# rgcgithub/regenie

Measured on NVIDIA H100. Metric: step1_level0_snps_per_sec, higher is better.
Workload: dtype int8 Gram + int8 prediction (both exact integer sums) + tf32x3 factorisation + f64 refinement / statistics

## Files before the change

### regenie_b200/csrc/chol_mixed.cu

```cuda
#include <algorithm>

#include "gemm_dmma.cuh"
#include "kernels.cuh"

namespace rg {

namespace {

constexpr int PT = 128;
constexpr int PLD = 132;
constexpr int PB = 32;
constexpr int kMxRowsPerCta = 64;

__device__ __forceinline__ void blk_nt(float (&acc)[PB], const float* __restrict__ Arow, const float* __restrict__ Bt, int plen) {
  for (int p0 = 0; p0 < plen; p0 += 4) {
    const float4 a = *reinterpret_cast<const float4*>(Arow + p0);
#pragma unroll
    for (int n = 0; n < PB; ++n) {
      const float4 b = *reinterpret_cast<const float4*>(Bt + n * PLD + p0);
      acc[n] = fmaf(a.x, b.x, acc[n]);
      acc[n] = fmaf(a.y, b.y, acc[n]);
      acc[n] = fmaf(a.z, b.z, acc[n]);
      acc[n] = fmaf(a.w, b.w, acc[n]);
    }
// ... 200 lines not shown
#pragma unroll
    for (int p = 0; p < PMAX; ++p) acc[a][p] = 0.0;
  double2 an2[4];
#pragma unroll
  for (int a = 0; a < 4; ++a) an2[a] = *reinterpret_cast<const double2*>(a0 + (int64_t)a * n + lane * 2);
  for (int j = lane * 2; j < n; j += 64) {
    double2 av[4];
#pragma unroll
    for (int a = 0; a < 4; ++a) av[a] = an2[a];
    if (j + 64 < n) {
#pragma unroll
      for (int a = 0; a < 4; ++a) an2[a] = *reinterpret_cast<const double2*>(a0 + (int64_t)a * n + j + 64);
    }
#pragma unroll
    for (int p = 0; p < PMAX; ++p) {
      if (p < P) {
        const double2 b = *reinterpret_cast<const double2*>(rs_sm + p * n + j);
#pragma unroll
        for (int a = 0; a < 4; ++a) acc[a][p] = fma(av[a].x, b.x, fma(av[a].y, b.y, acc[a][p]));
      }
    }
  }
#pragma unroll
  for (int a = 0; a < 4; ++a)
#pragma unroll
    for (int p = 0; p < PMAX; ++p) {
#pragma unroll
      for (int o = 16; o > 0; o >>= 1) acc[a][p] += __shfl_xor_sync(0xffffffffu, acc[a][p], o);
    }
  if (lane == 0) {
#pragma unroll
    for (int a = 0; a < 4; ++a)
#pragma unroll
      for (int p = 0; p < PMAX; ++p)
        if (p < P)
          rvec[((int64_t)m * Pp + p) * n + i0 + a] = bvec[((int64_t)f * Pp + p) * n + i0 + a] - lam * rs_sm[p * n + i0 + a] - acc[a][p];
  }
  }
}


constexpr int RF_ROWS = 64;
constexpr int RF_NV = 64;

__global__ void __launch_bounds__(256)
mx_residual_fused_kernel(const double* __restrict__ Af, const double* __restrict__ lambda, int R, const double* __restrict__ bvec,
                         const double* __restrict__ xvec, double* __restrict__ rvec, int n, int P, int Pp, int nmat, int step,
                         const unsigned int* __restrict__ conv, float tol) {
  __shared__ double As[64 * DM_LD], Bs[64 * DM_LD];
  const int f = blockIdx.y;
  if (step > 1) {
    bool all_done = true;
    for (int r = 0; r < R; ++r) all_done = all_done && mx_finished(conv, nmat, f * R + r, step - 1, tol);
    if (all_done) return;
  }
  const int NV = R * P;
  const int row0 = blockIdx.x * RF_ROWS;
  const int lrow = threadIdx.x >> 2, lp = (threadIdx.x & 3) * 4;
  const bool vb = lrow < NV;
  const double* ap = Af + ((int64_t)f * n + row0 + lrow) * n + lp;
  const double* bp = xvec + ((int64_t)(f * R + (vb ? lrow / P : 0)) * Pp + (vb ? lrow % P : 0)) * n + lp;
  DmmaAcc acc;
  gemm_tile_nt_dmma_ptr(ap, true, bp, vb, n, acc, As, Bs);
#pragma unroll
  for (int j = 0; j < 4; ++j)
#pragma unroll
    for (int e = 0; e < 2; ++e) {
      const int vec = dm_col(j) + e;
      if (vec < NV) {
        const int r = vec / P, p = vec % P, m = f * R + r;
        const double lam = lambda[r];
#pragma unroll
        for (int i = 0; i < 2; ++i) {
          const int row = row0 + dm_row(i);
          const int64_t o = ((int64_t)m * Pp + p) * n + row;
          rvec[o] = bvec[((int64_t)f * Pp + p) * n + row] - lam * xvec[o] - acc.c[i][j][e];
        }
      }
    }
}

constexpr int TS_STAGES = 6;
constexpr int TS_SUB = 32;
constexpr int TS_STAGE_BYTES = TS_SUB * PT * 4;
constexpr int TS_VP = 12;
constexpr int TS_CW = 16;

__device__ __forceinline__ uint32_t ts_smem_u32(const void* p) { return (uint32_t)__cvta_generic_to_shared(p); }
__device__ __forceinline__ void ts_mbar_wait(uint32_t bar, uint32_t parity) {
  uint32_t done = 0, spins = 0;
  while (true) {
    asm volatile(
        "{\n\t.reg .pred p;\n\t"
        "mbarrier.try_wait.parity.shared::cta.b64 p, [%1], %2;\n\t"
        "selp.u32 %0, 1, 0, p;\n\t}"
        : "=r"(done) : "r"(bar), "r"(parity) : "memory");
    if (done) break;
    if (++spins > (1u << 28)) __trap();
  }
}

template <int PMAX>
__global__ void __launch_bounds__(32 * (TS_CW + 1))
mx_trisolve_kernel(const __grid_constant__ CUtensorMap tmL, const __grid_constant__ CUtensorMap tmM,
                   const __grid_constant__ CUtensorMap tmMT, const double* __restrict__ rvec, int64_t r_mat_stride,
                   int r_mat_div, double* __restrict__ xvec, int n, int P, int Pp, int nmat, int step,
                   unsigned int* __restrict__ conv, float tol) {
  constexpr int TS_PARTS = TS_CW / 4;
  constexpr int TS_CPP = TS_SUB / TS_PARTS;
  constexpr int TS_THREADS = 32 * (TS_CW + 1);
  extern __shared__ uint8_t ts_raw[];
  const int m = blockIdx.x;
  if (step > 1 && mx_finished(conv, nmat, m, step - 1, tol)) return;
  const uint32_t raw = ts_smem_u32(ts_raw);
  const uint32_t base = (raw + 127u) & ~127u;
  uint8_t* gen = ts_raw + (base - raw);
  float* tiles = reinterpret_cast<float*>(gen);
  float* v = reinterpret_cast<float*>(gen + TS_STAGES * TS_STAGE_BYTES);
  float* sbuf = v + (size_t)n * TS_VP;
  float* comb = sbuf + PT * TS_VP;
  uint64_t* bars = reinterpret_cast<uint64_t*>(comb + (TS_PARTS - 1) * PT * TS_VP);
  const uint32_t full_bar = ts_smem_u32(bars), empty_bar = ts_smem_u32(bars + TS_STAGES);
  const int warp = threadIdx.x >> 5, lane = threadIdx.x & 31;
  const int nt = n / PT;
  if (threadIdx.x == 0) {
    for (int s = 0; s < TS_STAGES; ++s) {
      asm volatile("mbarrier.init.shared::cta.b64 [%0], %1;" ::"r"(full_bar + 8 * s), "r"(1) : "memory");
      asm volatile("mbarrier.init.shared::cta.b64 [%0], %1;" ::"r"(empty_bar + 8 * s), "r"(TS_CW) : "memory");
    }
    asm volatile("fence.mbarrier_init.release.cluster;" ::: "memory");
    asm volatile("fence.proxy.async.shared::cta;" ::: "memory");
  }
  const double* r = rvec + (int64_t)(r_mat_div > 0 ? m / r_mat_div : m) * r_mat_stride;
  for (int e = threadIdx.x; e < n * TS_VP; e += TS_THREADS) {
    const int i = e / TS_VP, p = e % TS_VP;
    v[e] = p < P ? (float)r[(int64_t)p * n + i] : 0.f;
  }
  __syncthreads();

  if (warp == TS_CW) {
    if (lane == 0) {
      asm volatile("prefetch.tensormap [%0];" ::"l"(&tmL) : "memory");
      asm volatile("prefetch.tensormap [%0];" ::"l"(&tmM) : "memory");
      asm volatile("prefetch.tensormap [%0];" ::"l"(&tmMT) : "memory");
      int it = 0;
      auto push = [&](const CUtensorMap* tm, int c0, int c1) {
        const int s = it % TS_STAGES;
        const uint32_t ph = (it / TS_STAGES) & 1;
        ts_mbar_wait(empty_bar + 8 * s, ph ^ 1);
        asm volatile("mbarrier.arrive.expect_tx.shared::cta.b64 _, [%0], %1;" ::"r"(full_bar + 8 * s), "r"(TS_STAGE_BYTES) : "memory");
        asm volatile(
            "cp.async.bulk.tensor.2d.shared::cluster.global.mbarrier::complete_tx::bytes [%0], [%1, {%3, %4}], [%2];"
            ::"r"(base + s * TS_STAGE_BYTES), "l"(tm), "r"(full_bar + 8 * s), "r"(c0), "r"(c1) : "memory");
        ++it;
      };
      for (int sweep = 0; sweep < 2; ++sweep)
        for (int kk = 0; kk < nt; ++kk) {
          const int k = sweep == 0 ? kk : nt - 1 - kk;
          const int j0 = sweep == 0 ? 0 : k + 1, j1 = sweep == 0 ? k : nt;
          for (int j = j0; j < j1; ++j)
            for (int sub = 0; sub < PT / TS_SUB; ++sub) push(&tmL, k * PT, m * n + j * PT + sub * TS_SUB);
          for (int sub = 0; sub < PT / TS_SUB; ++sub)
            push(sweep == 0 ? &tmMT : &tmM, 0, (m * nt + k) * PT + sub * TS_SUB);
        }
    }
    return;
  }

  const int half = warp >> 2;
  const int row = (warp & 3) * 32 + lane;
  int it = 0;
  float acc[PMAX];
  auto consume = [&](const float* vec ) {
    const int s = it % TS_STAGES;
    const uint32_t ph = (it / TS_STAGES) & 1;
    ts_mbar_wait(full_bar + 8 * s, ph);
    const float* t = tiles + (size_t)s * (TS_STAGE_BYTES / 4) + (size_t)(half * TS_CPP) * PT + row;
    const float* y = vec + (size_t)(half * TS_CPP) * TS_VP;
#pragma unroll
    for (int c = 0; c < TS_CPP; ++c) {
      const float tv = t[(size_t)c * PT];
      const float4 y0 = *reinterpret_cast<const float4*>(y + c * TS_VP);
      const float4 y1 = *reinterpret_cast<const float4*>(y + c * TS_VP + 4);
      const float4 y2 = *reinterpret_cast<const float4*>(y + c * TS_VP + 8);
      const float yy[12] = {y0.x, y0.y, y0.z, y0.w, y1.x, y1.y, y1.z, y1.w, y2.x, y2.y, y2.z, y2.w};
#pragma unroll
      for (int p = 0; p < PMAX; ++p) acc[p] = fmaf(tv, yy[p], acc[p]);
    }
    __syncwarp();
    if (lane == 0) asm volatile("mbarrier.arrive.shared::cta.b64 _, [%0];" ::"r"(empty_bar + 8 * s) : "memory");
    ++it;
  };
  auto consumer_sync = [&]() { asm volatile("bar.sync 1, %0;" ::"n"(32 * TS_CW) : "memory"); };

  for (int sweep = 0; sweep < 2; ++sweep)
    for (int kk = 0; kk < nt; ++kk) {
      const int k = sweep == 0 ? kk : nt - 1 - kk;
      const int j0 = sweep == 0 ? 0 : k + 1, j1 = sweep == 0 ? k : nt;
#pragma unroll
      for (int p = 0; p < PMAX; ++p) acc[p] = 0.f;
      for (int j = j0; j < j1; ++j)
        for (int sub = 0; sub < PT / TS_SUB; ++sub) consume(v + (size_t)(j * PT + sub * TS_SUB) * TS_VP);
      if (half > 0) {
#pragma unroll
        for (int p = 0; p < PMAX; ++p) comb[((half - 1) * PT + row) * TS_VP + p] = acc[p];
      }
      consumer_sync();
      if (half == 0) {
#pragma unroll
        for (int p = 0; p < PMAX; ++p) {
          float sum = acc[p];
#pragma unroll
          for (int h = 0; h < TS_PARTS - 1; ++h) sum += comb[(h * PT + row) * TS_VP + p];
          sbuf[row * TS_VP + p] = v[(size_t)(k * PT + row) * TS_VP + p] - sum;
        }
      }
      consumer_sync();
#pragma unroll
      for (int p = 0; p < PMAX; ++p) acc[p] = 0.f;
      for (int sub = 0; sub < PT / TS_SUB; ++sub) consume(sbuf + (size_t)(sub * TS_SUB) * TS_VP);
      if (half > 0) {
#pragma unroll
        for (int p = 0; p < PMAX; ++p) comb[((half - 1) * PT + row) * TS_VP + p] = acc[p];
      }
      consumer_sync();
      if (half == 0) {
#pragma unroll
        for (int p = 0; p < PMAX; ++p) {
          float sum = acc[p];
#pragma unroll
          for (int h = 0; h < TS_PARTS - 1; ++h) sum += comb[(h * PT + row) * TS_VP + p];
          v[(size_t)(k * PT + row) * TS_VP + p] = sum;
        }
      }
      consumer_sync();
    }

  float dmax = 0.f, xmax = 0.f;
  for (int e = threadIdx.x; e < P * n; e += 32 * TS_CW) {
    const int p = e / n, i = e % n;
    double* xp = xvec + ((int64_t)m * Pp + p) * n + i;
    const float dx = v[(size_t)i * TS_VP + p];
    const double xn = (step == 0 ? 0.0 : *xp) + (double)dx;
    *xp = xn;
    dmax = (fabsf(dx) <= 3.0e38f) ? fmaxf(dmax, fabsf(dx)) : __int_as_float(0x7f800000);
    xmax = fmaxf(xmax, fabsf((float)xn));
  }
  if (step > 0) {
#pragma unroll
    for (int o = 16; o > 0; o >>= 1) {
      dmax = fmaxf(dmax, __shfl_xor_sync(0xffffffffu, dmax, o));
      xmax = fmaxf(xmax, __shfl_xor_sync(0xffffffffu, xmax, o));
    }
    if (lane == 0) {
      atomicMax(conv + ((int64_t)step * nmat + m) * 2, __float_as_uint(dmax));
      atomicMax(conv + ((int64_t)step * nmat + m) * 2 + 1, __float_as_uint(xmax));
    }
  }
}

__global__ void mx_final_check_kernel(const unsigned int* __restrict__ conv, int nmat, int steps, float tol,
                                      unsigned int* __restrict__ fail_flag) {
  const int m = blockIdx.x * blockDim.x + threadIdx.x;
  if (m >= nmat) return;
  bool ok = mx_finished(conv, nmat, m, steps, tol);
  for (int s = 1; s <= steps; ++s) {
    const float dx = __uint_as_float(conv[((int64_t)s * nmat + m) * 2]);
    if (!(dx == dx) || !(fabsf(dx) <= 3.0e38f)) ok = false;
  }
  if (!ok) atomicOr(fail_flag, 1u);
}

struct MxPlan {
  int n = 0, nt = 0;
  DevBuf<int4> tiles;
  std::vector<int2> upd, trsm;
};

static void build_plan(MxPlan& pl, int n) {
  pl.n = n;
  const int nt = n / PT;
  pl.nt = nt;
  std::vector<int4> all;
  pl.upd.clear(); pl.trsm.clear();
  for (int k = 0; k < nt; ++k) {
    int2 u{(int)all.size(), 0};
    for (int i = k; i < nt; ++i) all.push_back(make_int4(i, k, 0, 4 * k));
    u.y = (int)all.size() - u.x;
    pl.upd.push_back(u);
    int2 t{(int)all.size(), 0};
    for (int i = k + 1; i < nt; ++i) all.push_back(make_int4(i, k, 4 * k, 4));
    t.y = (int)all.size() - t.x;
    pl.trsm.push_back(t);
  }
  pl.tiles.alloc(all.size());
  RG_CUDA(cudaMemcpy(pl.tiles.p, all.data(), all.size() * sizeof(int4), cudaMemcpyHostToDevice));
}

struct MixedSolver::Impl {
  int n = 0, nmat = 0, K = 0, R = 0, Pp = 0;
  DevBuf<float> Lplain, Mplain, MTplain, Ap;
  DevBuf<unsigned int> conv;
  CUtensorMap tmL, tmM, tmAp;
  CUtensorMap tmLpl, tmMpl, tmMTpl;
  MxPlan plan;
};

MixedSolver::MixedSolver() : impl(new Impl()) {}
MixedSolver::~MixedSolver() { delete impl; }

int MixedSolver::dim_for(int bs) {
  int n = PT;
  while (n < bs) n *= 2;
  return n <= 2048 ? n : 0;
}

void MixedSolver::prepare(int n, int K, int R, int Pp) {
  Impl& d = *impl;
  const int nmat = K * R;
  if (d.n == n && d.nmat == nmat && d.Pp == Pp) return;
  RG_CHECK(n % PT == 0 && n >= PT && ((n / PT) & (n / PT - 1)) == 0 && n <= 2048,
           "mixed solver: dimension must be 128 * 2^k <= 2048");
  d.n = n; d.nmat = nmat; d.K = K; d.R = R; d.Pp = Pp;
  d.Lplain.alloc((size_t)nmat * n * n);
  d.Mplain.alloc((size_t)nmat * n * PT);
  d.MTplain.alloc((size_t)nmat * n * PT);
  make_f32_rows_tensor_map(&d.tmLpl, d.Lplain.p, n, (int64_t)nmat * n, PT, TS_SUB);
  make_f32_rows_tensor_map(&d.tmMpl, d.Mplain.p, PT, (int64_t)nmat * n, PT, TS_SUB);
  make_f32_rows_tensor_map(&d.tmMTpl, d.MTplain.p, PT, (int64_t)nmat * n, PT, TS_SUB);
  RG_CUDA(cudaMemset(d.Lplain.p, 0, (size_t)nmat * n * n * 4));
  d.conv.alloc((size_t)(kMxMaxSteps + 1) * nmat * 2);
  make_tf32_operand_tensor_map(&d.tmL, d.Lplain.p, n, n, nmat);
  make_tf32_operand_tensor_map(&d.tmM, d.Mplain.p, PT, n, nmat);
  d.Ap.alloc((size_t)K * n * n);
  RG_CUDA(cudaMemset(d.Ap.p, 0, (size_t)K * n * n * 4));
  make_tf32_operand_tensor_map(&d.tmAp, d.Ap.p, n, n, K);
  build_plan(d.plan, n);
}

static int rhs_chunk(int n) { return std::max(1, std::min(12, (int)(98304 / (8 * (size_t)n)))); }

int MixedSolver::launches_per_solve(int n, int steps, int P) {
  const int nt = n / PT;
  const int nch = (P + rhs_chunk(n) - 1) / rhs_chunk(n);
  return 3 * nt - 1 + nch * (1 + 2 * steps) + 1;
}

void MixedSolver::solve(const double* Af, const double* lambda, const double* bvec, double* xvec, double* rvec, int P,
                        int steps, float tol, unsigned int* fail_flag, cudaStream_t s, bool first_col_ready) {
  Impl& d = *impl;
  const int n = d.n, nmat = d.nmat, nt = d.plan.nt;
  RG_CHECK(n > 0, "mixed solver: prepare() first");
  RG_CHECK(P <= d.Pp, "mixed solver: more right-hand sides than the row pitch");
  RG_CHECK(steps >= 1 && steps <= kMxMaxSteps, "mixed solver: bad step count");
  const size_t potrf_smem = ((size_t)3 * PT * PLD + PT + 2 * PB) * sizeof(float);
  ensure_dyn_smem(reinterpret_cast<const void*>(potrf128_kernel), potrf_smem);
  ensure_dyn_smem(reinterpret_cast<const void*>(mx_residual_kernel<12>), 98304);
  ensure_dyn_smem(reinterpret_cast<const void*>(mx_residual_kernel<10>), 98304);
  RG_CHECK(n <= 2048, "mixed solver: n <= 2048");
  const size_t sm_t = (size_t)TS_STAGES * TS_STAGE_BYTES + ((size_t)n + (1 + TS_CW / 4) * PT) * TS_VP * sizeof(float) + 2 * TS_STAGES * 8 + 256;
  ensure_dyn_smem(reinterpret_cast<const void*>(mx_trisolve_kernel<12>), sm_t);
  ensure_dyn_smem(reinterpret_cast<const void*>(mx_trisolve_kernel<10>), sm_t);
  RG_CUDA(cudaMemsetAsync(d.conv.p, 0, d.conv.n * sizeof(unsigned int), s));
  const int4* tl = d.plan.tiles.p;
  Tf32GemmEpilogue e0{};
  e0.n = n; e0.out_mat_stride = (int64_t)n * n; e0.out = d.Lplain.p;
  for (int k = 0; k < nt; ++k) {
    Tf32GemmEpilogue e = e0;
    e.c_chunks = 4; e.c_mat_div = d.R;
    e.diag_add = lambda; e.diag_mod = d.R;
    if (!(k == 0 && first_col_ready)) launch_tf32x3_gemm(d.tmL, d.tmL, tl + d.plan.upd[k].x, d.plan.upd[k].y, nmat, e, s, &d.tmAp);
    potrf128_kernel<<<nmat, 256, potrf_smem, s>>>(d.Lplain.p, d.Mplain.p, d.MTplain.p, n, k, fail_flag);
    if (d.plan.trsm[k].y > 0) {
      Tf32GemmEpilogue t = e0;
      t.mirror = 1;
      t.b_cols_local = 1;
      launch_tf32x3_gemm(d.tmL, d.tmM, tl + d.plan.trsm[k].x, d.plan.trsm[k].y, nmat, t, s);
    }
  }
  dim3 grid(n / kMxRowsPerCta, nmat);
  const int pc = rhs_chunk(n);
  for (int st = 0; st <= steps; ++st)
    for (int p0 = 0; p0 < P; p0 += pc) {
      const int np = std::min(pc, P - p0);
      const size_t sm_r = (size_t)np * n * sizeof(double);
      const int64_t o = (int64_t)p0 * n;
      auto tri = [&](const double* rv, int64_t rs, int rdiv, int step) {
#define RG_TRI(PM) mx_trisolve_kernel<PM><<<nmat, 32 * (TS_CW + 1), sm_t, s>>>(d.tmLpl, d.tmMpl, d.tmMTpl, rv, rs, rdiv, xvec + o, n, np, d.Pp, nmat, step, d.conv.p, tol)
        if (np <= 10) RG_TRI(10);
        else RG_TRI(12);
#undef RG_TRI
      };
      if (st == 0) {
        tri(bvec + o, (int64_t)d.Pp * n, d.R, 0);
      } else {
        if (d.R * np <= RF_NV && n % RF_ROWS == 0)
          mx_residual_fused_kernel<<<dim3(n / RF_ROWS, d.K), 256, 0, s>>>(Af, lambda, d.R, bvec + o, xvec + o, rvec + o, n, np, d.Pp, nmat, st, d.conv.p, tol);
        else if (np <= 10) mx_residual_kernel<10><<<grid, 256, sm_r, s>>>(Af, lambda, d.R, bvec + o, xvec + o, rvec + o, n, np, d.Pp, nmat, st, d.conv.p, tol);
        else mx_residual_kernel<12><<<grid, 256, sm_r, s>>>(Af, lambda, d.R, bvec + o, xvec + o, rvec + o, n, np, d.Pp, nmat, st, d.conv.p, tol);
        tri(rvec + o, (int64_t)d.Pp * n, 0, st);
      }
    }
  mx_final_check_kernel<<<(nmat + 63) / 64, 64, 0, s>>>(d.conv.p, nmat, steps, tol, fail_flag);
}

float* MixedSolver::a_planes() { return impl->Ap.p; }
float* MixedSolver::l_planes() { return impl->Lplain.p; }

const float* MixedSolver::debug_planes(int which) const {
  switch (which) {
    case 2: return impl->Lplain.p;
    case 3: return impl->Mplain.p;
    default: return nullptr;
  }
}

}
```

### regenie_b200/csrc/kernels.cuh

```cuda
#pragma once
#include "common.cuh"

namespace rg {

constexpr int kMaxFolds = 16;
constexpr int kMaxCov = 64;
constexpr int kMaxRidge = 8;
constexpr int kMaxPhenoTile = 8;
constexpr int kLimbs = 9;
constexpr int kLimbsI8 = 5;
constexpr int kLimbQI8 = 50;

void launch_partial_sum(const double* part, int nchunks, int64_t per, double* out, cudaStream_t s);

__device__ __forceinline__ uint32_t miss_bits(uint32_t w) { return w & (w >> 1) & 0x55555555u; }
struct BedMissOut {
  const int4* ctile = nullptr;
  int nct = 0;
  int rows_p = 0;
  unsigned long long* total = nullptr;
  unsigned long long cap = 0;
  int2* seg = nullptr;
  int32_t* list = nullptr;
  uint32_t* gt = nullptr;
// ... 20 lines not shown
  double *gty_f, *rhs;
  unsigned long long* err_slot;
  long long err_base;
};

struct AssembleArgs {
  int bs, rows_p, nC, C, K, R, loocv;
  const float* zz;
  int64_t ldz, zz_fold_stride;
  const double *mu, *inv_sd, *Bv, *Af, *Qf;
  const double* lambda;
  double* cm;
  int64_t cm_stride;
  int ldc;
  float* planes = nullptr;
  float* lplanes = nullptr;
};

void launch_l0_stats(const uint32_t* gp, int64_t npad, const double* xy, int cpp, const int4* chunks,
                     int nchunks, int rows_p, int32_t* cnt_part, double* sum_part, cudaStream_t s);
void launch_l0_fold_reduce(const int32_t* cnt_part, const double* sum_part, int rows_p, int cpp,
                           const int2* fold_chunks, int K, int32_t* cnt_fold, double* sum_fold,
                           cudaStream_t s);
void launch_l0_snp_finalize(const SnpFinalizeArgs& a, cudaStream_t s);
void launch_l0_assemble(const AssembleArgs& a, const double* rhs, int P, int Ppad, int nmat, cudaStream_t s);

void make_gram_tensor_map(CUtensorMap* tm, const uint8_t* z, int64_t npad, int rows2);
constexpr int kStatQ = 14;
constexpr int kStatOnesRow = 126;
void launch_l0_xy_digits(const double* xy, int cpp, int ncol, int64_t npad, const uint8_t* is_real, double* scale,
                         uint8_t* D, cudaStream_t s);
void launch_l0_stats_finish(const float* T, int ldt, int64_t t_fold_stride, const float* zz, int ldz,
                            int64_t zz_fold_stride, int rows_p, int cpp, int ncol, int K, const double* scale,
                            int32_t* cnt_fold, double* sum_fold, cudaStream_t s);
void gram_tile_list(int rows2, std::vector<int2>& tiles);
void stat_tile_list(int zrows, int drows, int bn, std::vector<int2>& tiles);
struct ZPlanes {
  uint32_t lut[3];
};
constexpr uint32_t kPlaneG = 0x00100800u;
constexpr uint32_t kPlaneG2 = 0x00200800u;
constexpr uint32_t kPlaneMiss = 0x08000000u;
constexpr ZPlanes kZLevel0 = {{kPlaneG, kPlaneMiss, 0u}};
constexpr ZPlanes kZStep2 = {{kPlaneG, kPlaneG2, kPlaneMiss}};
void launch_gram_gp(const CUtensorMap& tmG, const CUtensorMap* tmD, int rows_p, const ZPlanes& planes,
                    const int2* tiles, int ntiles, const int2* fold_k, int K, float* out, int ldo, int64_t fold_stride,
                    float out_scale, cudaStream_t s, int bn = 256, const unsigned long long* miss_total = nullptr,
                    int64_t miss_cap = 0, int miss_tile0 = 0);
constexpr float kZScaleGram = 1.f / 64;
constexpr float kZScaleStat = 1.f / 8;
constexpr double kMissSparseRate = 0.015;
void launch_miss_sparse(const uint32_t* gt, int rows_p, const int2* seg, int nct, const int2* fold_ct,
                        const int32_t* list, int K, const unsigned long long* total, int64_t cap, float* zz,
                        int64_t fold_stride, cudaStream_t s);
void launch_gram_reference(const uint32_t* gp, int64_t npad, int rows_p, int k0, int k1, float* out, int ldo,
                           cudaStream_t s);

void launch_chol_factor(double* cm, int64_t stride, int nC, int n_aug, int batch, double* inv,
                        unsigned long long* err_slot, long long err_base, cudaStream_t s);
void launch_chol_backsolve(double* cm, int64_t stride, int nC, int P, int batch, const double* inv,
                           cudaStream_t s);
int chol_num_launches(int nC);
size_t chol_inv_elems(int nC, int batch);
void launch_chol_rows_backsolve(double* cm, int64_t stride, int nC, int row0, int nrows, int batch,
                                const double* inv, cudaStream_t s);

struct Tf32GemmEpilogue {
  int n;
  int64_t out_mat_stride;
  float* out;
  int mirror;
  int b_cols_local;
  int negate;
  int lower_only;
  const double* cin;
  int64_t cin_mat_stride;
  int cin_ld, cin_mat_div;
  const double* diag_add;
  int diag_mod;
  int c_chunks;
  int c_mat_div;
};
void make_tf32_operand_tensor_map(CUtensorMap* tm, const float* base, int cols, int rows, int batch);
void make_f32_rows_tensor_map(CUtensorMap* tm, const float* base, int cols, int64_t rows, int box_cols, int box_rows);
void launch_tf32x3_gemm(const CUtensorMap& tmA, const CUtensorMap& tmB, const int4* tiles, int ntiles, int batch,
                        const Tf32GemmEpilogue& ep, cudaStream_t s, const CUtensorMap* tmC = nullptr);

constexpr int kMxMaxSteps = 6;
class MixedSolver {
 public:
  MixedSolver();
  ~MixedSolver();
  MixedSolver(const MixedSolver&) = delete;
  MixedSolver& operator=(const MixedSolver&) = delete;
  static int dim_for(int bs);
  void prepare(int n, int K, int R, int Pp);
  float* a_planes();
  float* l_planes();
  void solve(const double* Af, const double* lambda, const double* bvec, double* xvec, double* rvec, int P, int steps,
             float tol, unsigned int* fail_flag, cudaStream_t s, bool first_col_ready = false);
  static int launches_per_solve(int n, int steps, int P);
  const float* debug_planes(int which) const;
 private:
  struct Impl;
  Impl* impl;
};
void launch_l0_assemble_sym(const AssembleArgs& a, const double* rhs, int P, int Pp, double* bvec, cudaStream_t s);

void launch_dense_from_dosage(const uint8_t* probs, const uint8_t* miss, int64_t n_file, int bs, const int32_t* file_idx_pad,
                              int ref_first, double* gd, int64_t npad, cudaStream_t s);
void launch_dense_from_f64(const double* G, int64_t n_file, int bs, const int32_t* file_idx_pad, double* gd, int64_t npad,
                           cudaStream_t s);
void launch_dense_prepare(double* gd, int64_t npad, int bs, const int32_t* file_idx_pad, const double* xy, int cpp, int C,
                          long long n_analyzed, double numtol, double* mu, double* inv_sd, unsigned long long* err_slot,
                          long long err_base, cudaStream_t s);
void launch_dense_predict(const double* gd, int64_t npad, int bs, const double* cm, int64_t cm_stride, int ldc, int nC, int R,
                          int P, const int32_t* tile_fold, const uint8_t* mask, double* const* W, int col0, cudaStream_t s);

struct PredictArgs {
  int bs, rows_p, C, P, R, Qp, cpp, col0;
  int64_t npad, words_per_row;
  const uint32_t* gp;
  const int32_t* tile_fold;
  const double *gam, *gmu;
  const double* cvec;
  const double* xy;
  const uint8_t* mask;
  double* const* W;
  double* part;
};
void launch_l0_gamma(const double* cm, int64_t cm_stride, int ldc, int nC, int R, int P, int Qp,
                     int bs, int rows_p, int K, const double* mu, const double* inv_sd,
                     const double* Bv, int C, double* gam, double* gmu, double* cvec, cudaStream_t s);
void launch_l0_predict(const PredictArgs& a, int ntiles, cudaStream_t s);
void launch_l0_standardize(const double* part, int ntiles, int Qp, int Q, int P, const double* neff,
                           double* mean_invsd, double* const* W, int64_t npad, int col0,
                           const uint8_t* is_real, cudaStream_t s, const double* const* src = nullptr, int src_col0 = 0);
int predict_qt();

struct PredictTcArgs {
  int rows_p, C, P, Q, Qp, cpp, col0, ngroups;
  int64_t npad;
  const int32_t* tile_fold;
  const double* scale;
  const double* cvec;
  const double* xy;
  const uint8_t* mask;
  double* const* W;
  double* part;
};
void make_byte_tensor_map(CUtensorMap* tm, const uint8_t* basep, int64_t inner, int64_t rows);
void make_gp_tensor_map(CUtensorMap* tm, const uint32_t* gp, int64_t words_per_row, int64_t rows);
int launch_l0_colsum(double* const* W, int64_t npad, int col0, int P, int Q, int Qp, double* part,
                     cudaStream_t s);
size_t predict_i8_dig_bytes(int K, int ngroups, int rows_p);
void launch_l0_coef_i8(const double* cm, int64_t cm_stride, int ldc, int nC, int R, int P, int Q, int Qp, int bs,
                       int rows_p, int K, const double* mu, const double* inv_sd, const double* Bv, int C, double* gam,
                       double* gmu, double* cvec, double* scale, uint8_t* dig, int ngroups, cudaStream_t s);
void launch_l0_predict_i8(const CUtensorMap& tmG, const CUtensorMap& tmD, const PredictTcArgs& a, int ntiles,
                          cudaStream_t s);

void launch_l1_gram(const double* W, int64_t ldw, int B, const int4* chunks, int nchunks, double* part,
                    int64_t part_stride, int ldp, cudaStream_t s);
void launch_l1_xty(const double* W, int64_t ldw, const double* xy, int cpp, int ycol, const int4* chunks,
                   int nchunks, double* part_y, int B, cudaStream_t s);
void launch_l1_assemble(const double* part, int64_t part_stride, int ldp, const double* part_y, int64_t part_y_stride,
                        int P, const int2* fold_chunks, int K, int R1, const double* tau, int B, int nC, double* cm,
// ... 313 lines not shown
```

### regenie_b200/csrc/tf32_gemm.cu

```cuda
#include "kernels.cuh"
#include "wgmma_sm90.cuh"

namespace rg {

namespace {

using namespace sm90;

constexpr int TG_M = 128, TG_N = 128;
constexpr int TG_KC = 32;
constexpr int TG_STAGES = 2;
constexpr int TG_TILE_BYTES = TG_M * 128;
constexpr int TG_STAGE_BYTES = 2 * TG_TILE_BYTES;
constexpr int TG_LO_OFF = TG_STAGES * TG_STAGE_BYTES;
constexpr int TG_SMEM_BYTES = TG_LO_OFF + TG_STAGE_BYTES;
constexpr int TG_THREADS = 160;

__device__ __forceinline__ float4 tf32_rn4(const float4 v) {
  uint4 t;
  asm("cvt.rna.tf32.f32 %0, %1;" : "=r"(t.x) : "f"(v.x));
  asm("cvt.rna.tf32.f32 %0, %1;" : "=r"(t.y) : "f"(v.y));
  asm("cvt.rna.tf32.f32 %0, %1;" : "=r"(t.z) : "f"(v.z));
  asm("cvt.rna.tf32.f32 %0, %1;" : "=r"(t.w) : "f"(v.w));
  return make_float4(__uint_as_float(t.x), __uint_as_float(t.y), __uint_as_float(t.z), __uint_as_float(t.w));
// ... 161 lines not shown
    const double* cin = ep.cin ? ep.cin + (int64_t)(ep.cin_mat_div > 0 ? mat / ep.cin_mat_div : mat) * ep.cin_mat_stride + (int64_t)row * ep.cin_ld + col0
                               : nullptr;
    const double diag_add = (ep.diag_add != nullptr && tile.x == tile.y) ? ep.diag_add[ep.diag_mod > 0 ? mat % ep.diag_mod : mat] : 0.0;
    const bool diag_tile = tile.x == tile.y;
    float* st = reinterpret_cast<float*>(gen_base) + (size_t)q * (32 * TG_N) + (size_t)lane * TG_N;
    constexpr int EC = 16;
#pragma unroll 1
    for (int c = 0; c < TG_N / EC; ++c) {
      float v[EC];
#pragma unroll
      for (int j = 0; j < EC; j += 4) {
        const float4 t4 = *reinterpret_cast<const float4*>(st + 4 * (((c * EC + j) >> 2) ^ lane));
        v[j] = t4.x; v[j + 1] = t4.y; v[j + 2] = t4.z; v[j + 3] = t4.w;
      }
      float o[EC];
      if (cin) {
#pragma unroll
        for (int j = 0; j < EC; j += 2) {
          const double2 cc = *reinterpret_cast<const double2*>(cin + c * EC + j);
          o[j] = (float)(cc.x - (double)v[j]);
          o[j + 1] = (float)(cc.y - (double)v[j + 1]);
        }
      } else {
#pragma unroll
        for (int j = 0; j < EC; ++j) o[j] = ep.negate ? -v[j] : v[j];
      }
      if (diag_tile && diag_add != 0.0) {
#pragma unroll
        for (int j = 0; j < EC; ++j) if (c * EC + j == r_loc) o[j] = (float)((double)o[j] + diag_add);
      }
      if (ep.lower_only && diag_tile) {
#pragma unroll
        for (int j = 0; j < EC; ++j) if (c * EC + j > r_loc) o[j] = 0.f;
      }
#pragma unroll
      for (int j = 0; j < EC; j += 4) {
        const int chunk = (c * EC + j) >> 2;
        *reinterpret_cast<float4*>(st + 4 * (chunk ^ lane)) = make_float4(o[j], o[j + 1], o[j + 2], o[j + 3]);
      }
      if (ep.mirror && !diag_tile) {
        float* pt = ep.out + mat_off + (int64_t)(col0 + c * EC) * n + row;
#pragma unroll
        for (int j = 0; j < EC; ++j) pt[(int64_t)j * n] = o[j];
      }
    }
    __syncwarp();
    {
      const float* stw = reinterpret_cast<const float*>(gen_base) + (size_t)q * (32 * TG_N);
      float* po = ep.out + mat_off + (int64_t)(tile.x * TG_M + q * 32) * n + col0 + lane * 4;
#pragma unroll 4
      for (int rr = 0; rr < 32; ++rr)
        *reinterpret_cast<float4*>(po + (int64_t)rr * n) = *reinterpret_cast<const float4*>(stw + (size_t)rr * TG_N + 4 * (lane ^ rr));
    }
  }
}

typedef CUresult (*EncodeTiledFn)(CUtensorMap*, CUtensorMapDataType, cuuint32_t, void*, const cuuint64_t*,
                                  const cuuint64_t*, const cuuint32_t*, const cuuint32_t*, CUtensorMapInterleave,
                                  CUtensorMapSwizzle, CUtensorMapL2promotion, CUtensorMapFloatOOBfill);

static EncodeTiledFn tg_encode_fn() {
  static EncodeTiledFn fn = nullptr;
  if (!fn) {
    void* p = nullptr;
    cudaDriverEntryPointQueryResult qres;
    RG_CUDA(cudaGetDriverEntryPoint("cuTensorMapEncodeTiled", &p, cudaEnableDefault, &qres));
    RG_CHECK(p != nullptr && qres == cudaDriverEntryPointSuccess, "cuTensorMapEncodeTiled not available");
    fn = reinterpret_cast<EncodeTiledFn>(p);
  }
  return fn;
}

void make_tf32_operand_tensor_map(CUtensorMap* tm, const float* base, int cols, int rows, int batch) {
  const cuuint64_t gdim[3] = {(cuuint64_t)cols, (cuuint64_t)rows, (cuuint64_t)batch};
  const cuuint64_t gstride[2] = {(cuuint64_t)cols * 4, (cuuint64_t)rows * cols * 4};
  const cuuint32_t box[3] = {TG_KC, 128, 1};
  const cuuint32_t estr[3] = {1, 1, 1};
  CUresult r = tg_encode_fn()(tm, CU_TENSOR_MAP_DATA_TYPE_FLOAT32, 3, const_cast<float*>(base), gdim, gstride, box, estr,
                              CU_TENSOR_MAP_INTERLEAVE_NONE, CU_TENSOR_MAP_SWIZZLE_128B, CU_TENSOR_MAP_L2_PROMOTION_L2_256B,
                              CU_TENSOR_MAP_FLOAT_OOB_FILL_NONE);
  RG_CHECK(r == CUDA_SUCCESS, "cuTensorMapEncodeTiled (tf32 operand) failed (" + std::to_string((int)r) + ")");
}

void make_f32_rows_tensor_map(CUtensorMap* tm, const float* base, int cols, int64_t rows, int box_cols, int box_rows) {
  const cuuint64_t gdim[2] = {(cuuint64_t)cols, (cuuint64_t)rows};
  const cuuint64_t gstride[1] = {(cuuint64_t)cols * 4};
  const cuuint32_t box[2] = {(cuuint32_t)box_cols, (cuuint32_t)box_rows};
  const cuuint32_t estr[2] = {1, 1};
  CUresult r = tg_encode_fn()(tm, CU_TENSOR_MAP_DATA_TYPE_FLOAT32, 2, const_cast<float*>(base), gdim, gstride, box, estr,
                              CU_TENSOR_MAP_INTERLEAVE_NONE, CU_TENSOR_MAP_SWIZZLE_NONE, CU_TENSOR_MAP_L2_PROMOTION_L2_256B,
                              CU_TENSOR_MAP_FLOAT_OOB_FILL_NONE);
  RG_CHECK(r == CUDA_SUCCESS, "cuTensorMapEncodeTiled (f32 rows) failed (" + std::to_string((int)r) + ")");
}

void launch_tf32x3_gemm(const CUtensorMap& tmA, const CUtensorMap& tmB, const int4* tiles, int ntiles, int batch,
                        const Tf32GemmEpilogue& ep, cudaStream_t s, const CUtensorMap* tmC) {
  RG_CHECK(ep.c_chunks == 0 || tmC, "tf32 gemm: the C phase needs its tensor map");
  RG_CHECK(ep.out != nullptr, "tf32 gemm: no output");
  if (ntiles <= 0 || batch <= 0) return;
  const size_t smem = (size_t)TG_SMEM_BYTES + 1024 + 128;
  dim3 grid(ntiles, batch);
  ensure_dyn_smem(reinterpret_cast<const void*>(tf32x3_gemm_nt_kernel), smem);
  tf32x3_gemm_nt_kernel<<<grid, TG_THREADS, smem, s>>>(tmA, tmB, tmC ? *tmC : tmA, tiles, ep);
}

}
```

Measured before the change: 1.036 million.

## Move mixed-precision triangular solve inner products onto tf32x3 mma.sync tensor cores

Rewrites the blocked triangular solve consumer so that tile-by-vector products use m16n8k8 tf32 mma.sync with a three-product hi/lo split instead of scalar FMAs. Leftover right-hand-side columns beyond 8 stay on FMAs with shuffle reductions. The TMA loads now use 128B-swizzled 32-column boxes, and the solution vector uses an XOR-swizzled layout to match the mma fragments. Consumer warps drop from 16 to 8, which removes the cross-warp combine buffer and one barrier per block step. Blocks of the diagonal tile that cannot contribute are skipped. The risks are lower per-CTA parallelism and a small change in accuracy from the tf32x3 products.

```diff
diff --git a/regenie_b200/csrc/chol_mixed.cu b/regenie_b200/csrc/chol_mixed.cu
--- a/regenie_b200/csrc/chol_mixed.cu
+++ b/regenie_b200/csrc/chol_mixed.cu
@@ -306,9 +306,9 @@
 
 constexpr int TS_STAGES = 6;
 constexpr int TS_SUB = 32;
+constexpr int TS_BOX = 32;
 constexpr int TS_STAGE_BYTES = TS_SUB * PT * 4;
-constexpr int TS_VP = 12;
-constexpr int TS_CW = 16;
+constexpr int TS_CW = 8;
 
 __device__ __forceinline__ uint32_t ts_smem_u32(const void* p) { return (uint32_t)__cvta_generic_to_shared(p); }
 __device__ __forceinline__ void ts_mbar_wait(uint32_t bar, uint32_t parity) {
@@ -324,26 +324,83 @@
   }
 }
 
-template <int PMAX>
-__global__ void __launch_bounds__(32 * (TS_CW + 1))
+template <int VW>
+__device__ __forceinline__ int ts_vidx(int i, int p) {
+  const int q = i >> 1;
+  return q * 2 * VW + 2 * (p ^ (4 * ((q * VW / 16) & (VW / 4 - 1)))) + (i & 1);
+}
+
+__device__ __forceinline__ void ts_split(float x, uint32_t& hi, uint32_t& lo) {
+  hi = (__float_as_uint(x) + 0x1000u) & 0xffffe000u;
+  lo = __float_as_uint(x - __uint_as_float(hi));
+}
+
+__device__ __forceinline__ void ts_mma(float (&d)[4], const uint32_t (&a)[4], uint32_t b0, uint32_t b1) {
+  asm("mma.sync.aligned.m16n8k8.row.col.f32.tf32.tf32.f32 {%0, %1, %2, %3}, {%4, %5, %6, %7}, {%8, %9}, {%0, %1, %2, %3};"
+      : "+f"(d[0]), "+f"(d[1]), "+f"(d[2]), "+f"(d[3])
+      : "r"(a[0]), "r"(a[1]), "r"(a[2]), "r"(a[3]), "r"(b0), "r"(b1));
+}
+
+template <int NF>
+__device__ __forceinline__ void ts_consume(float (&acc)[4][4], float (&accf)[2][NF > 0 ? NF : 1], const float* tiles,
+                                           const float* vec, const int (&aoff)[4], int boff, const int (&foff)[NF > 0 ? NF : 1],
+                                           uint32_t full_bar, uint32_t empty_bar, int it, int lane, bool live) {
+  constexpr int VW = NF > 0 ? 16 : 8;
+  const int s = it % TS_STAGES;
+  const uint32_t ph = (it / TS_STAGES) & 1;
+  ts_mbar_wait(full_bar + 8 * s, ph);
+  const float* st = tiles + (size_t)s * (TS_STAGE_BYTES / 4);
+  if (live)
+#pragma unroll
+  for (int kc = 0; kc < TS_SUB / 8; ++kc) {
+    float a[4];
+    uint32_t ahi[4], alo[4];
+#pragma unroll
+    for (int q = 0; q < 4; ++q) {
+      a[q] = st[aoff[q] + kc * 8 * TS_BOX];
+      ts_split(a[q], ahi[q], alo[q]);
+    }
+    const float2 b = *reinterpret_cast<const float2*>(vec + boff + kc * 8 * VW);
+    uint32_t bh0, bl0, bh1, bl1;
+    ts_split(b.x, bh0, bl0);
+    ts_split(b.y, bh1, bl1);
+    const int c = 2 * (kc & 1);
+    ts_mma(acc[c], alo, bh0, bh1);
+    ts_mma(acc[c], ahi, bl0, bl1);
+    ts_mma(acc[c + 1], ahi, bh0, bh1);
+#pragma unroll
+    for (int f = 0; f < NF; ++f) {
+      const float2 y = *reinterpret_cast<const float2*>(vec + foff[f] + kc * 8 * VW);
+      accf[0][f] = fmaf(a[2], y.y, fmaf(a[0], y.x, accf[0][f]));
+      accf[1][f] = fmaf(a[3], y.y, fmaf(a[1], y.x, accf[1][f]));
+    }
+  }
+  __syncwarp();
+  if (lane == 0) asm volatile("mbarrier.arrive.shared::cta.b64 _, [%0];" ::"r"(empty_bar + 8 * s) : "memory");
+}
+
+__device__ __forceinline__ float ts_sum(const float (&acc)[4][4], int e) {
+  return (acc[1][e] + acc[3][e]) + (acc[0][e] + acc[2][e]);
+}
+
+template <int NF>
+__global__ void __launch_bounds__(32 * (TS_CW + 1), 1)
 mx_trisolve_kernel(const __grid_constant__ CUtensorMap tmL, const __grid_constant__ CUtensorMap tmM,
                    const __grid_constant__ CUtensorMap tmMT, const double* __restrict__ rvec, int64_t r_mat_stride,
                    int r_mat_div, double* __restrict__ xvec, int n, int P, int Pp, int nmat, int step,
                    unsigned int* __restrict__ conv, float tol) {
-  constexpr int TS_PARTS = TS_CW / 4;
-  constexpr int TS_CPP = TS_SUB / TS_PARTS;
-  constexpr int TS_THREADS = 32 * (TS_CW + 1);
+  constexpr int VW = NF > 0 ? 16 : 8;
+  constexpr int NFA = NF > 0 ? NF : 1;
   extern __shared__ uint8_t ts_raw[];
   const int m = blockIdx.x;
   if (step > 1 && mx_finished(conv, nmat, m, step - 1, tol)) return;
   const uint32_t raw = ts_smem_u32(ts_raw);
-  const uint32_t base = (raw + 127u) & ~127u;
+  const uint32_t base = (raw + 1023u) & ~1023u;
   uint8_t* gen = ts_raw + (base - raw);
   float* tiles = reinterpret_cast<float*>(gen);
   float* v = reinterpret_cast<float*>(gen + TS_STAGES * TS_STAGE_BYTES);
-  float* sbuf = v + (size_t)n * TS_VP;
-  float* comb = sbuf + PT * TS_VP;
-  uint64_t* bars = reinterpret_cast<uint64_t*>(comb + (TS_PARTS - 1) * PT * TS_VP);
+  float* sbuf = v + (size_t)n * VW;
+  uint64_t* bars = reinterpret_cast<uint64_t*>(sbuf + PT * VW);
   const uint32_t full_bar = ts_smem_u32(bars), empty_bar = ts_smem_u32(bars + TS_STAGES);
   const int warp = threadIdx.x >> 5, lane = threadIdx.x & 31;
   const int nt = n / PT;
@@ -354,11 +411,6 @@
     }
     asm volatile("fence.mbarrier_init.release.cluster;" ::: "memory");
     asm volatile("fence.proxy.async.shared::cta;" ::: "memory");
-  }
-  const double* r = rvec + (int64_t)(r_mat_div > 0 ? m / r_mat_div : m) * r_mat_stride;
-  for (int e = threadIdx.x; e < n * TS_VP; e += TS_THREADS) {
-    const int i = e / TS_VP, p = e % TS_VP;
-    v[e] = p < P ? (float)r[(int64_t)p * n + i] : 0.f;
   }
   __syncthreads();
 
@@ -373,9 +425,12 @@
         const uint32_t ph = (it / TS_STAGES) & 1;
         ts_mbar_wait(empty_bar + 8 * s, ph ^ 1);
         asm volatile("mbarrier.arrive.expect_tx.shared::cta.b64 _, [%0], %1;" ::"r"(full_bar + 8 * s), "r"(TS_STAGE_BYTES) : "memory");
-        asm volatile(
-            "cp.async.bulk.tensor.2d.shared::cluster.global.mbarrier::complete_tx::bytes [%0], [%1, {%3, %4}], [%2];"
-            ::"r"(base + s * TS_STAGE_BYTES), "l"(tm), "r"(full_bar + 8 * s), "r"(c0), "r"(c1) : "memory");
+#pragma unroll
+        for (int b = 0; b < PT / TS_BOX; ++b)
+          asm volatile(
+              "cp.async.bulk.tensor.2d.shared::cluster.global.mbarrier::complete_tx::bytes [%0], [%1, {%3, %4}], [%2];"
+              ::"r"(base + s * TS_STAGE_BYTES + b * TS_SUB * TS_BOX * 4), "l"(tm), "r"(full_bar + 8 * s),
+                "r"(c0 + b * TS_BOX), "r"(c1) : "memory");
         ++it;
       };
       for (int sweep = 0; sweep < 2; ++sweep)
@@ -391,80 +446,104 @@
     return;
   }
 
-  const int half = warp >> 2;
-  const int row = (warp & 3) * 32 + lane;
+  auto consumer_sync = [&]() { asm volatile("bar.sync 1, %0;" ::"n"(32 * TS_CW) : "memory"); };
+  const double* r = rvec + (int64_t)(r_mat_div > 0 ? m / r_mat_div : m) * r_mat_stride;
+#pragma unroll 4
+  for (int e = threadIdx.x; e < n * VW; e += 32 * TS_CW) {
+    const int p = e / n, i = e % n;
+    v[ts_vidx<VW>(i, p)] = p < P ? (float)r[(int64_t)p * n + i] : 0.f;
+  }
+  consumer_sync();
+  const int g = lane >> 2, t = lane & 3;
+  int aoff[4];
+#pragma unroll
+  for (int q = 0; q < 4; ++q) {
+    const int c = 2 * t + (q >> 1);
+    const int rr = 16 * (warp & 1) + g + 8 * (q & 1);
+    aoff[q] = (warp >> 1) * TS_SUB * TS_BOX + c * TS_BOX + ((((rr >> 2) ^ c) & 7) << 2) + (rr & 3);
+  }
+  const int boff = ts_vidx<VW>(2 * t, g);
+  int foff[NFA];
+#pragma unroll
+  for (int f = 0; f < NFA; ++f) foff[f] = ts_vidx<VW>(2 * t, 8 + f);
   int it = 0;
-  float acc[PMAX];
-  auto consume = [&](const float* vec ) {
-    const int s = it % TS_STAGES;
-    const uint32_t ph = (it / TS_STAGES) & 1;
-    ts_mbar_wait(full_bar + 8 * s, ph);
-    const float* t = tiles + (size_t)s * (TS_STAGE_BYTES / 4) + (size_t)(half * TS_CPP) * PT + row;
-    const float* y = vec + (size_t)(half * TS_CPP) * TS_VP;
-#pragma unroll
-    for (int c = 0; c < TS_CPP; ++c) {
-      const float tv = t[(size_t)c * PT];
-      const float4 y0 = *reinterpret_cast<const float4*>(y + c * TS_VP);
-      const float4 y1 = *reinterpret_cast<const float4*>(y + c * TS_VP + 4);
-      const float4 y2 = *reinterpret_cast<const float4*>(y + c * TS_VP + 8);
-      const float yy[12] = {y0.x, y0.y, y0.z, y0.w, y1.x, y1.y, y1.z, y1.w, y2.x, y2.y, y2.z, y2.w};
-#pragma unroll
-      for (int p = 0; p < PMAX; ++p) acc[p] = fmaf(tv, yy[p], acc[p]);
-    }
-    __syncwarp();
-    if (lane == 0) asm volatile("mbarrier.arrive.shared::cta.b64 _, [%0];" ::"r"(empty_bar + 8 * s) : "memory");
-    ++it;
+  float acc[4][4], accf[2][NFA];
+  auto consume = [&](const float* vec, bool live) {
+    ts_consume<NF>(acc, accf, tiles, vec, aoff, boff, foff, full_bar, empty_bar, it++, lane, live);
   };
-  auto consumer_sync = [&]() { asm volatile("bar.sync 1, %0;" ::"n"(32 * TS_CW) : "memory"); };
+  auto zero = [&]() {
+#pragma unroll
+    for (int c = 0; c < 4; ++c)
+#pragma unroll
+      for (int e = 0; e < 4; ++e) acc[c][e] = 0.f;
+#pragma unroll
+    for (int f = 0; f < NFA; ++f) accf[0][f] = accf[1][f] = 0.f;
+  };
+  const int row0 = 16 * warp + g;
+  auto fsum = [&](float (&out)[2][NFA]) {
+#pragma unroll
+    for (int h = 0; h < 2; ++h)
+#pragma unroll
+      for (int f = 0; f < NF; ++f) {
+        float x = accf[h][f];
+        x += __shfl_xor_sync(0xffffffffu, x, 1);
+        x += __shfl_xor_sync(0xffffffffu, x, 2);
+        out[h][f] = x;
+      }
+  };
 
   for (int sweep = 0; sweep < 2; ++sweep)
     for (int kk = 0; kk < nt; ++kk) {
       const int k = sweep == 0 ? kk : nt - 1 - kk;
       const int j0 = sweep == 0 ? 0 : k + 1, j1 = sweep == 0 ? k : nt;
-#pragma unroll
-      for (int p = 0; p < PMAX; ++p) acc[p] = 0.f;
+      zero();
       for (int j = j0; j < j1; ++j)
-        for (int sub = 0; sub < PT / TS_SUB; ++sub) consume(v + (size_t)(j * PT + sub * TS_SUB) * TS_VP);
-      if (half > 0) {
-#pragma unroll
-        for (int p = 0; p < PMAX; ++p) comb[((half - 1) * PT + row) * TS_VP + p] = acc[p];
+        for (int sub = 0; sub < PT / TS_SUB; ++sub) consume(v + (size_t)(j * PT + sub * TS_SUB) * VW, true);
+#pragma unroll
+      for (int e = 0; e < 4; ++e) {
+        const int row = row0 + 8 * (e >> 1), p = 2 * t + (e & 1);
+        sbuf[ts_vidx<VW>(row, p)] = v[ts_vidx<VW>(k * PT + row, p)] - ts_sum(acc, e);
+      }
+      if (NF > 0) {
+        float fs[2][NFA];
+        fsum(fs);
+#pragma unroll
+        for (int f = 0; f < NF; ++f)
+          if (t == f) {
+#pragma unroll
+            for (int h = 0; h < 2; ++h)
+              sbuf[ts_vidx<VW>(row0 + 8 * h, 8 + f)] = v[ts_vidx<VW>(k * PT + row0 + 8 * h, 8 + f)] - fs[h][f];
+          }
       }
       consumer_sync();
-      if (half == 0) {
-#pragma unroll
-        for (int p = 0; p < PMAX; ++p) {
-          float sum = acc[p];
-#pragma unroll
-          for (int h = 0; h < TS_PARTS - 1; ++h) sum += comb[(h * PT + row) * TS_VP + p];
-          sbuf[row * TS_VP + p] = v[(size_t)(k * PT + row) * TS_VP + p] - sum;
-        }
+      zero();
+      for (int sub = 0; sub < PT / TS_SUB; ++sub)
+        consume(sbuf + (size_t)(sub * TS_SUB) * VW,
+                sweep == 0 ? 16 * warp + 15 >= sub * TS_SUB : 16 * warp <= sub * TS_SUB + TS_SUB - 1);
+#pragma unroll
+      for (int e = 0; e < 4; ++e) {
+        const int row = row0 + 8 * (e >> 1), p = 2 * t + (e & 1);
+        v[ts_vidx<VW>(k * PT + row, p)] = ts_sum(acc, e);
+      }
+      if (NF > 0) {
+        float fs[2][NFA];
+        fsum(fs);
+#pragma unroll
+        for (int f = 0; f < NF; ++f)
+          if (t == f) {
+#pragma unroll
+            for (int h = 0; h < 2; ++h) v[ts_vidx<VW>(k * PT + row0 + 8 * h, 8 + f)] = fs[h][f];
+          }
       }
       consumer_sync();
-#pragma unroll
-      for (int p = 0; p < PMAX; ++p) acc[p] = 0.f;
-      for (int sub = 0; sub < PT / TS_SUB; ++sub) consume(sbuf + (size_t)(sub * TS_SUB) * TS_VP);
-      if (half > 0) {
-#pragma unroll
-        for (int p = 0; p < PMAX; ++p) comb[((half - 1) * PT + row) * TS_VP + p] = acc[p];
-      }
-      consumer_sync();
-      if (half == 0) {
-#pragma unroll
-        for (int p = 0; p < PMAX; ++p) {
-          float sum = acc[p];
-#pragma unroll
-          for (int h = 0; h < TS_PARTS - 1; ++h) sum += comb[(h * PT + row) * TS_VP + p];
-          v[(size_t)(k * PT + row) * TS_VP + p] = sum;
-        }
-      }
-      consumer_sync();
     }
 
   float dmax = 0.f, xmax = 0.f;
+#pragma unroll 4
   for (int e = threadIdx.x; e < P * n; e += 32 * TS_CW) {
     const int p = e / n, i = e % n;
     double* xp = xvec + ((int64_t)m * Pp + p) * n + i;
-    const float dx = v[(size_t)i * TS_VP + p];
+    const float dx = v[ts_vidx<VW>(i, p)];
     const double xn = (step == 0 ? 0.0 : *xp) + (double)dx;
     *xp = xn;
     dmax = (fabsf(dx) <= 3.0e38f) ? fmaxf(dmax, fabsf(dx)) : __int_as_float(0x7f800000);
@@ -549,9 +628,9 @@
   d.Lplain.alloc((size_t)nmat * n * n);
   d.Mplain.alloc((size_t)nmat * n * PT);
   d.MTplain.alloc((size_t)nmat * n * PT);
-  make_f32_rows_tensor_map(&d.tmLpl, d.Lplain.p, n, (int64_t)nmat * n, PT, TS_SUB);
-  make_f32_rows_tensor_map(&d.tmMpl, d.Mplain.p, PT, (int64_t)nmat * n, PT, TS_SUB);
-  make_f32_rows_tensor_map(&d.tmMTpl, d.MTplain.p, PT, (int64_t)nmat * n, PT, TS_SUB);
+  make_f32_rows_tensor_map(&d.tmLpl, d.Lplain.p, n, (int64_t)nmat * n, TS_BOX, TS_SUB, true);
+  make_f32_rows_tensor_map(&d.tmMpl, d.Mplain.p, PT, (int64_t)nmat * n, TS_BOX, TS_SUB, true);
+  make_f32_rows_tensor_map(&d.tmMTpl, d.MTplain.p, PT, (int64_t)nmat * n, TS_BOX, TS_SUB, true);
   RG_CUDA(cudaMemset(d.Lplain.p, 0, (size_t)nmat * n * n * 4));
   d.conv.alloc((size_t)(kMxMaxSteps + 1) * nmat * 2);
   make_tf32_operand_tensor_map(&d.tmL, d.Lplain.p, n, n, nmat);
@@ -582,9 +661,15 @@
   ensure_dyn_smem(reinterpret_cast<const void*>(mx_residual_kernel<12>), 98304);
   ensure_dyn_smem(reinterpret_cast<const void*>(mx_residual_kernel<10>), 98304);
   RG_CHECK(n <= 2048, "mixed solver: n <= 2048");
-  const size_t sm_t = (size_t)TS_STAGES * TS_STAGE_BYTES + ((size_t)n + (1 + TS_CW / 4) * PT) * TS_VP * sizeof(float) + 2 * TS_STAGES * 8 + 256;
-  ensure_dyn_smem(reinterpret_cast<const void*>(mx_trisolve_kernel<12>), sm_t);
-  ensure_dyn_smem(reinterpret_cast<const void*>(mx_trisolve_kernel<10>), sm_t);
+  const int pc = rhs_chunk(n);
+  auto sm_tri = [&](int nf) {
+    return (size_t)TS_STAGES * TS_STAGE_BYTES + ((size_t)n + PT) * (nf > 0 ? 16 : 8) * sizeof(float) + 2 * TS_STAGES * 8 + 1024;
+  };
+  ensure_dyn_smem(reinterpret_cast<const void*>(mx_trisolve_kernel<0>), sm_tri(0));
+  if (pc > 8) {
+    ensure_dyn_smem(reinterpret_cast<const void*>(mx_trisolve_kernel<2>), sm_tri(2));
+    ensure_dyn_smem(reinterpret_cast<const void*>(mx_trisolve_kernel<4>), sm_tri(4));
+  }
   RG_CUDA(cudaMemsetAsync(d.conv.p, 0, d.conv.n * sizeof(unsigned int), s));
   const int4* tl = d.plan.tiles.p;
   Tf32GemmEpilogue e0{};
@@ -603,16 +688,16 @@
     }
   }
   dim3 grid(n / kMxRowsPerCta, nmat);
-  const int pc = rhs_chunk(n);
   for (int st = 0; st <= steps; ++st)
     for (int p0 = 0; p0 < P; p0 += pc) {
       const int np = std::min(pc, P - p0);
       const size_t sm_r = (size_t)np * n * sizeof(double);
       const int64_t o = (int64_t)p0 * n;
       auto tri = [&](const double* rv, int64_t rs, int rdiv, int step) {
-#define RG_TRI(PM) mx_trisolve_kernel<PM><<<nmat, 32 * (TS_CW + 1), sm_t, s>>>(d.tmLpl, d.tmMpl, d.tmMTpl, rv, rs, rdiv, xvec + o, n, np, d.Pp, nmat, step, d.conv.p, tol)
-        if (np <= 10) RG_TRI(10);
-        else RG_TRI(12);
+#define RG_TRI(NF) mx_trisolve_kernel<NF><<<nmat, 32 * (TS_CW + 1), sm_tri(NF), s>>>(d.tmLpl, d.tmMpl, d.tmMTpl, rv, rs, rdiv, xvec + o, n, np, d.Pp, nmat, step, d.conv.p, tol)
+        if (np <= 8) RG_TRI(0);
+        else if (np <= 10) RG_TRI(2);
+        else RG_TRI(4);
 #undef RG_TRI
       };
       if (st == 0) {
diff --git a/regenie_b200/csrc/kernels.cuh b/regenie_b200/csrc/kernels.cuh
--- a/regenie_b200/csrc/kernels.cuh
+++ b/regenie_b200/csrc/kernels.cuh
@@ -126,7 +126,8 @@
   int c_mat_div;
 };
 void make_tf32_operand_tensor_map(CUtensorMap* tm, const float* base, int cols, int rows, int batch);
-void make_f32_rows_tensor_map(CUtensorMap* tm, const float* base, int cols, int64_t rows, int box_cols, int box_rows);
+void make_f32_rows_tensor_map(CUtensorMap* tm, const float* base, int cols, int64_t rows, int box_cols, int box_rows,
+                              bool swizzle_128b);
 void launch_tf32x3_gemm(const CUtensorMap& tmA, const CUtensorMap& tmB, const int4* tiles, int ntiles, int batch,
                         const Tf32GemmEpilogue& ep, cudaStream_t s, const CUtensorMap* tmC = nullptr);
 
diff --git a/regenie_b200/csrc/tf32_gemm.cu b/regenie_b200/csrc/tf32_gemm.cu
--- a/regenie_b200/csrc/tf32_gemm.cu
+++ b/regenie_b200/csrc/tf32_gemm.cu
@@ -267,14 +267,15 @@
   RG_CHECK(r == CUDA_SUCCESS, "cuTensorMapEncodeTiled (tf32 operand) failed (" + std::to_string((int)r) + ")");
 }
 
-void make_f32_rows_tensor_map(CUtensorMap* tm, const float* base, int cols, int64_t rows, int box_cols, int box_rows) {
+void make_f32_rows_tensor_map(CUtensorMap* tm, const float* base, int cols, int64_t rows, int box_cols, int box_rows,
+                              bool swizzle_128b) {
   const cuuint64_t gdim[2] = {(cuuint64_t)cols, (cuuint64_t)rows};
   const cuuint64_t gstride[1] = {(cuuint64_t)cols * 4};
   const cuuint32_t box[2] = {(cuuint32_t)box_cols, (cuuint32_t)box_rows};
   const cuuint32_t estr[2] = {1, 1};
   CUresult r = tg_encode_fn()(tm, CU_TENSOR_MAP_DATA_TYPE_FLOAT32, 2, const_cast<float*>(base), gdim, gstride, box, estr,
-                              CU_TENSOR_MAP_INTERLEAVE_NONE, CU_TENSOR_MAP_SWIZZLE_NONE, CU_TENSOR_MAP_L2_PROMOTION_L2_256B,
-                              CU_TENSOR_MAP_FLOAT_OOB_FILL_NONE);
+                              CU_TENSOR_MAP_INTERLEAVE_NONE, swizzle_128b ? CU_TENSOR_MAP_SWIZZLE_128B : CU_TENSOR_MAP_SWIZZLE_NONE,
+                              CU_TENSOR_MAP_L2_PROMOTION_L2_256B, CU_TENSOR_MAP_FLOAT_OOB_FILL_NONE);
   RG_CHECK(r == CUDA_SUCCESS, "cuTensorMapEncodeTiled (f32 rows) failed (" + std::to_string((int)r) + ")");
 }
 
```

Result: no change. 1.036 million, median of 6 (+0.0%).
